# ORNL/MultiDistTorch

Measured on AMD Instinct MI355X. Metric: aggregate VAE samples/sec across K concurrent HPO trials, higher is better.
Workload: dtype bf16; 1 GPU; model=conv-VAE 28x28 (2 conv + 2 deconv, z=32), global_batch=128, per_trial_batch=128, image=28, parallelism=groups1x1, trials=1, backend=hip, graphs=True, timing_barrier=none, valid=True

## Files before the change

csrc/kernels/common.h:

```cpp
#pragma once
#include <hip/hip_runtime.h>
#include <stdint.h>

namespace mdt {

typedef float f32x4 __attribute__((ext_vector_type(4)));
typedef float f32x16 __attribute__((ext_vector_type(16)));

constexpr int kWave = 64;

__device__ __forceinline__ int lane_id() { return threadIdx.x & 63; }
__device__ __forceinline__ int wave_id() { return threadIdx.x >> 6; }

__device__ __forceinline__ f32x4 mfma16x16x4(float a, float b, f32x4 c) {
  return __builtin_amdgcn_mfma_f32_16x16x4f32(a, b, c, 0, 0, 0);
}

__device__ __forceinline__ f32x16 mfma32x32x2(float a, float b, f32x16 c) {
  return __builtin_amdgcn_mfma_f32_32x32x2f32(a, b, c, 0, 0, 0);
}

__device__ __forceinline__ float wave_sum(float v) {
#pragma unroll
  for (int o = 32; o > 0; o >>= 1) v += __shfl_xor(v, o, 64);
// ... 43 lines not shown
#pragma clang fp contract(off)
  return 1.f + lv - mu * mu - sd * sd;
}
__device__ __forceinline__ bool fb_clamped(float sum, float fb) { return fb > 0.f && -0.5f * sum < fb; }
__device__ __forceinline__ float fb_fwd(float sum, float fb) { return fb_clamped(sum, fb) ? -2.f * fb : sum; }
__device__ __forceinline__ float fb_bwd(float sum, float fb, float beta) { return fb_clamped(sum, fb) ? 0.f : beta; }

__device__ __forceinline__ float kl_dmu(float dz, float be, float mu) { return fmaf(be, mu, dz); }
__device__ __forceinline__ float kl_dlv(float dz, float ep, float sd, float be) {
  return fmaf(sd, 0.5f * dz * ep, 0.5f * be * fmaf(sd, sd, -1.f));
}
__device__ __forceinline__ float kl_dlv_sum(float dz, float ep, float sd, float be) {
  return fmaf(0.5f * be, fmaf(sd, sd, -1.f), 0.5f * dz * ep * sd);
}

__device__ __forceinline__ void st_wt8(void* p, unsigned long long v) {
  __hip_atomic_store(reinterpret_cast<unsigned long long*>(p), v, __ATOMIC_RELAXED, __HIP_MEMORY_SCOPE_AGENT);
}

__device__ __forceinline__ bool p2p_wait_abandoned(const int* status, const int* abort_flag, int lane) {
  int bad = 0;
  if (lane == 0) {
    bad = __hip_atomic_load(status, __ATOMIC_RELAXED, __HIP_MEMORY_SCOPE_SYSTEM) != 0;
    if (!bad && abort_flag) bad = __hip_atomic_load(abort_flag, __ATOMIC_RELAXED, __HIP_MEMORY_SCOPE_SYSTEM) != 0;
  }
  return __any(bad);
}

}
```

csrc/kernels/conv28_pair.h:

```cpp
#pragma once
#include <stddef.h>

#include "conv28_fused.h"

namespace mdt {
namespace f28 {

struct PairCtl {
  unsigned long long* xg;
  int* pairw;
  unsigned* err;
  int M;
  int pair;
  int delay_us;
  int acquire;
  AdamC* adamc;
};

constexpr int kX1 = 0, kX2 = 72, kX3 = kX2 + 800, kX4 = kX3 + 784, kX5 = kX4 + 1568, kX6 = kX5 + 32;
constexpr int kXW = kX6 + 800;
constexpr unsigned long long kSpinTicks = 25000000ull;

enum : int { kModeSolo = 0, kModeRole0 = 1, kModeRole1 = 2, kModeExit = 3 };

// ... 41 lines not shown
    if (!__any(pend != 0)) break;
    if ((spin & 15) == 15 && __builtin_amdgcn_s_memrealtime() - t0 > kSpinTicks) {
      if (pend) atomicOr(err, 1u);
      break;
    }
    __builtin_amdgcn_s_sleep(1);
  }
#pragma unroll
  for (int k = 0; k < N; ++k)
    if (gi[k] >= 0) {
      if (near && MDT_F28_NEAR_WG)
        __hip_atomic_store((g64*)(base + gi[k]), 0ull, __ATOMIC_RELAXED, __HIP_MEMORY_SCOPE_WORKGROUP);
      else
        __hip_atomic_store((g64*)(base + gi[k]), 0ull, __ATOMIC_RELAXED, __HIP_MEMORY_SCOPE_AGENT);
    }
}

using kseg = const __attribute__((address_space(4))) char;
__device__ __forceinline__ kseg* kargs() {
  kseg* k = (kseg*)__builtin_amdgcn_kernarg_segment_ptr();
  asm volatile("" : "+s"(k));
  return k;
}

template <class T>
__device__ __forceinline__ T kval(size_t off) {
  return *(const __attribute__((address_space(4))) T*)(kargs() + off);
}

template <class T>
__device__ __forceinline__ T* kptr(size_t off, size_t stride = 0, int n = 0) {
  const unsigned long long v = kval<unsigned long long>(off);
  auto* g = (__attribute__((address_space(1))) T*)(v ? v + stride * (unsigned long long)n : 0ull);
  return (T*)g;
}
#define F28_KP(T, member, stride) kptr<T>(offsetof(StepKargs, member), (stride), n)

__device__ __forceinline__ uint32_t fbits(float f) { return __builtin_bit_cast(uint32_t, f); }
__device__ __forceinline__ float bitsf(uint32_t u) { return __builtin_bit_cast(float, u); }
__device__ __forceinline__ uint32_t bf16bits(__bf16 h) { return (uint32_t)__builtin_bit_cast(uint16_t, h); }

template <class BFrag, class Pre, class Epi>
// ... 667 lines not shown
```

csrc/kernels/conv_bf16.hip:

```cpp
#include <stdlib.h>
#include "common.h"
#include "vae_mlp.h"
#include "adam_common.h"
#include "conv_igemm.h"
#include "conv_small.h"

namespace mdt {

__global__ void __launch_bounds__(256) reparam_k(const float* mulv, float* eps, __bf16* z16, float* z32, int B,
                                                 int Z, const TrainState* st, const HParams* hp, uint32_t stream,
                                                 float* kld_part) {
  __shared__ float scratch[16];
  const int e = blockIdx.x * blockDim.x + threadIdx.x;
  float kl = 0.f;
  if (e < B * Z) {
    const int i = e / Z, c = e - i * Z;
    const float mu = mulv[(size_t)i * 2 * Z + c], lv = mulv[(size_t)i * 2 * Z + Z + c];
    const long long stp = st->step - 1;
    const float fb = st->fb_t;
    const u32x4 bits = philox4x32_10(u32x4{(uint32_t)(i * Z + c), stream, (uint32_t)((unsigned long long)stp & 0xffffffffu),
                                           (uint32_t)((unsigned long long)stp >> 32)},
                                     hp->seed_lo, hp->seed_hi);
    const float ep = normal_from_bits(bits.x, bits.y);
    const float sd = expf(0.5f * lv);
// ... 196 lines not shown
int mdt_adam_cast(float* P, const float* G, float* Mo, float* Vo, void* w16, const void* segs, int nseg,
                  long long total, const void* st, const void* hp, int do_adam, hipStream_t s) {
  (void)segs;
  (void)nseg;
  if (total % 4 || ((uintptr_t)P | (uintptr_t)G | (uintptr_t)Mo | (uintptr_t)Vo) % 16 || (uintptr_t)w16 % 8) return 1;
  int blocks = cdivh(total / 4, 256);
  if (blocks > 1024) blocks = 1024;
  if (blocks < 1) blocks = 1;
  hipLaunchKernelGGL(adam_cast_k, dim3(blocks), dim3(256), 0, s, P, G, Mo, Vo, reinterpret_cast<__bf16*>(w16), total,
                     reinterpret_cast<const TrainState*>(st), reinterpret_cast<const HParams*>(hp), do_adam);
  return (int)hipGetLastError();
}

int mdt_grad_finalize(float* P, float* G, float* Mo, float* Vo, void* w16, const void* segs, const void* units,
                      int nunits, const void* st, const void* hp, int do_adam, const float* gX, const int* gidx,
                      float* xn, unsigned* xtag, int gB, hipStream_t s) {
  if (nunits <= 0) return 0;
  const FinalizeArgs fa{P, G, Mo, Vo, reinterpret_cast<__bf16*>(w16), reinterpret_cast<const GradSeg*>(segs),
                        reinterpret_cast<const GradUnit*>(units), reinterpret_cast<const TrainState*>(st),
                        reinterpret_cast<const HParams*>(hp), do_adam};
  const bool gather = xn && xtag && gX && gidx && gB > 0;
  const BatchGather bg{gX, gidx, reinterpret_cast<const TrainState*>(st), gather ? xn : nullptr, xtag, gB, nunits};
  const int grid = nunits + (gather ? gather_blocks(gB) : 0);
  static const bool fence = [] {
    const char* e = getenv("MDT_FIN_FENCE");
    return e && e[0] == '1';
  }();
  if (fence)
    hipLaunchKernelGGL(grad_finalize_k<true>, dim3(grid), dim3(kFinalizeThreads), 0, s, fa, bg);
  else
    hipLaunchKernelGGL(grad_finalize_k<false>, dim3(grid), dim3(kFinalizeThreads), 0, s, fa, bg);
  return (int)hipGetLastError();
}

int mdt_wtrans(const void* w16, void* w16t, const void* segs, const void* units, int nunits, hipStream_t s) {
// ... 29 lines not shown
```

csrc/kernels/conv_jobs.hip:

```cpp
#include <string.h>

#include <algorithm>

#include "conv_direct.h"
#include "conv_dwgrad.h"
#include "conv_igemm_dev.h"
#include "comm_jobs.h"
#include "conv_small.h"
#include "conv_thin.h"
#include "conv_thin_wg.h"

namespace mdt {
using namespace tiles;

struct JobPack {
  JobBlob j[3];
  int start1, start2;
};

template <class T>
__device__ __forceinline__ const T& job_args(const JobBlob& j) {
  return *reinterpret_cast<const T*>(j.args);
}

// ... 133 lines not shown
    case kJobWgradAdam:
      wgrad_body<__bf16, true, W0, true>(job_args<WgAdamArgs>(j).w, lds, lb, j.nblk, &job_args<WgAdamArgs>(j));
      break;
    case kJobWgradAdam + 1:
      wgrad_body<__bf16, true, W1, true>(job_args<WgAdamArgs>(j).w, lds, lb, j.nblk, &job_args<WgAdamArgs>(j));
      break;
    case kJobLossStep: JLossStep::run(j, lds, lb); break;
    case kJobLoss: JLoss::run(j, lds, lb); break;
    case kJobFinalize: JFinalize::run(j, lds, lb); break;
    case kJobComm: JComm::run(j, lds, lb); break;
    case kJobColsum: JColsum::run(j, lds, lb); break;
    default: break;
  }
}

__global__ void __launch_bounds__(256) jobs_multi_k(const JobPackN* __restrict__ p) {
  __shared__ __attribute__((aligned(16))) uint8_t lds[kMultiLds];
  const int b = blockIdx.x;
  int st[kMaxMultiJobs];
#pragma unroll
  for (int k = 0; k < kMaxMultiJobs; ++k) st[k] = p->start[k];
  const int n = p->n;
  int i = 0, s0 = st[0];
#pragma unroll
  for (int k = 1; k < kMaxMultiJobs; ++k)
    if (k < n && b >= st[k]) {
      i = k;
      s0 = st[k];
    }
  unsigned long long* stamps = p->stamps;
  unsigned long long t0 = 0;
  if (stamps) t0 = __builtin_amdgcn_s_memrealtime();
  run_multi_job(p->j[i], lds, b - s0);
  if (stamps) {
    __syncthreads();
    if (threadIdx.x == 0) {
      stamps[2 * b] = t0;
      stamps[2 * b + 1] = __builtin_amdgcn_s_memrealtime();
    }
  }
}

__host__ inline bool multi_kind_ok(int k) {
  if (k >= kJobWgrad && k <= kJobWgrad + 5) return true;
  if (k >= kJobWgradThin && k <= kJobWgradThin + 5) return true;
  if (k >= kJobWgradThin + 20 && k <= kJobWgradThin + 25) return true;
  if (k == kJobWgradAdam || k == kJobWgradAdam + 1) return true;
  return k == kJobLossStep || k == kJobLoss || k == kJobFinalize || k == kJobColsum || k == kJobComm;
}

template <class A, class B, class C>
__global__ void __launch_bounds__(256) jobs_k(JobPack p) {
  __shared__ __attribute__((aligned(1024))) uint8_t lds[cmax(cmax(A::LDS, B::LDS), cmax(C::LDS, 16))];
  const int b = blockIdx.x;
  if (b < p.start1) A::run(p.j[0], lds, b);
// ... 226 lines not shown
  return 0;
}

int mdt_job_loss(JobBlob* j, const float* bce_part, int nb, const float* kld_part, int nk, void* st, const void* hp,
                 int advance_cursor) {
  memset(j, 0, sizeof(*j));
  j->kind = (advance_cursor & 2) ? kJobLossStep : kJobLoss;
  advance_cursor &= 1;
  j->nblk = 1;
  put_args(j, LossArgs{bce_part, nb, kld_part, nk, reinterpret_cast<TrainState*>(st),
                       reinterpret_cast<const HParams*>(hp), advance_cursor});
  return 0;
}

int mdt_job_finalize(JobBlob* j, float* P, float* G, float* Mo, float* Vo, void* w16, const void* segs,
                     const void* units, int nunits, const void* st, const void* hp, int do_adam) {
  memset(j, 0, sizeof(*j));
  if (nunits <= 0) return 1;
  j->kind = kJobFinalize;
  j->nblk = nunits;
  put_args(j, FinalizeArgs{P, G, Mo, Vo, reinterpret_cast<__bf16*>(w16), reinterpret_cast<const GradSeg*>(segs),
                           reinterpret_cast<const GradUnit*>(units), reinterpret_cast<const TrainState*>(st),
                           reinterpret_cast<const HParams*>(hp), do_adam});
  return 0;
}

int mdt_job_comm(JobBlob* j, float* P, float* G, float* Mo, float* Vo, void* w16, const void* segs, const void* units,
                 int nunits, const void* st, const void* hp, int do_adam, const void* ctx, int mode) {
  memset(j, 0, sizeof(*j));
  if (nunits <= 0 || !ctx || mode < kCommPush || mode > kCommPushReduce) return 1;
  j->kind = kJobComm;
  j->nblk = nunits;
  CommJobArgs a{};
  a.fa = FinalizeArgs{P, G, Mo, Vo, reinterpret_cast<__bf16*>(w16), reinterpret_cast<const GradSeg*>(segs),
                      reinterpret_cast<const GradUnit*>(units), reinterpret_cast<const TrainState*>(st),
                      reinterpret_cast<const HParams*>(hp), do_adam};
  a.ctx = reinterpret_cast<const CommCtx*>(ctx);
  a.mode = mode;
  put_args(j, a);
  return 0;
}

int mdt_job_wtrans(JobBlob* j, const void* w16, void* w16t, const void* segs, const void* units, int nunits) {
  memset(j, 0, sizeof(*j));
  if (nunits <= 0) return 1;
  j->kind = kJobWtrans;
  j->nblk = nunits;
  put_args(j, WtransArgs{reinterpret_cast<const __bf16*>(w16), reinterpret_cast<__bf16*>(w16t),
                         reinterpret_cast<const GradSeg*>(segs), reinterpret_cast<const TrUnit*>(units)});
  return 0;
}
// ... 40 lines not shown
    p.start[i] = grid;
    grid += jobs[i].nblk;
  }
  p.start[n] = grid;
  p.n = n;
  memcpy(dst, &p, sizeof(p));
  return grid;
}

int mdt_launch_jobs_multi(const void* dev_pack, int grid, hipStream_t s) {
  if (!dev_pack || grid <= 0) return 2;
  hipLaunchKernelGGL(jobs_multi_k, dim3(grid), dim3(256), 0, s, reinterpret_cast<const JobPackN*>(dev_pack));
  return (int)hipGetLastError() ? -1 : 0;
}

int mdt_launch_job1(const JobBlob* j, hipStream_t s) {
  if (j->kind == kJobCombine) return launch_splitk_combine(*reinterpret_cast<const CombineArgs*>(j->args), j->nblk, s);
  return 1;
}

}
```

csrc/kernels/conv_small.h:

```cpp
#pragma once
#include "adam_common.h"
#include "common.h"
#include "conv_igemm.h"
#include "vae_mlp.h"

namespace mdt {

struct LossArgs {
  const float* bce_part;
  int nb;
  const float* kld_part;
  int nk;
  TrainState* st;
  const HParams* hp;
  int advance_cursor;
};

__device__ __forceinline__ void loss_finalize_body(const LossArgs& la, float* scratch) {
  float sb = 0.f, sk = 0.f;
  for (int i = threadIdx.x; i < la.nb; i += blockDim.x) sb += la.bce_part[i];
  for (int i = threadIdx.x; i < la.nk; i += blockDim.x) sk += la.kld_part[i];
  const float bce = block_sum(sb, scratch);
  __syncthreads();
  const float kld = block_sum(sk, scratch);
// ... 240 lines not shown
  a.dmulv[(size_t)i * 2 * a.Z + a.Z + c] = dl;
  if (a.dmulv16) {
    a.dmulv16[(size_t)i * 2 * a.Z + c] = (__bf16)dm;
    a.dmulv16[(size_t)i * 2 * a.Z + a.Z + c] = (__bf16)dl;
  }
}

struct FinalizeArgs {
  float *P, *G, *Mo, *Vo;
  __bf16* w16;
  const GradSeg* segs;
  const GradUnit* units;
  const TrainState* st;
  const HParams* hp;
  int do_adam;
};

constexpr int kFinalizeThreads = 256;

struct BatchGather {
  const float* X;
  const int* idx;
  const TrainState* st;
  float* xn;
  unsigned* xtag;
  int B, nunits;
};
__host__ __device__ constexpr int gather_blocks(int B) { return (B * 196 + kFinalizeThreads - 1) / kFinalizeThreads; }

__device__ __forceinline__ void batch_gather_body(const BatchGather& g, int b) {
// ... 86 lines not shown
    if (sg.slab) {
      g = slab_sum1(sg.slab + e0 + j, n, sg.nsplit);
      if (!a.do_adam) a.G[o + j] = g;
    } else {
      g = a.G[o + j];
    }
    if (a.do_adam) {
      float p = a.P[o + j], m = a.Mo[o + j], v = a.Vo[o + j];
      adam_update(p, m, v, g, c);
      a.P[o + j] = p; a.Mo[o + j] = m; a.Vo[o + j] = v;
      a.w16[o + j] = (__bf16)p;
    }
  }
}

__device__ __forceinline__ void grad_finalize_body(const FinalizeArgs& a, float* red, AdamC* cs, int bid) {
  AdamC c{};
  if (a.do_adam) c = adam_consts_block(a.st, a.hp, cs);
  const GradUnit u = a.units[bid];
  const GradSeg sg = a.segs[u.seg];
  if (u.count > kFinalizeThreads) {
    grad_finalize_vec4(a, c, u, sg);
    return;
  }
  const int t = threadIdx.x, cnt = u.count, rp = kFinalizeThreads / cnt;
  const int col = t % cnt, rl = t / cnt;
  float part = 0.f;
  if (sg.slab && rl < rp) part = slab_partial(sg.slab + u.start + col, sg.numel, sg.nsplit, rl, rp);
  red[t] = part;
  __syncthreads();
  if (rl == 0) {
    const long long o = sg.off + u.start + col;
    float g;
    if (sg.slab) {
      g = 0.f;
// ... 71 lines not shown
```

csrc/runtime/conv_ops.cpp:

```cpp
#include <torch/extension.h>
#include <c10/hip/HIPStream.h>
#include <ATen/hip/impl/HIPGuardImplMasqueradingAsCUDA.h>

#include <cmath>
#include <cstring>
#include <tuple>
#include <vector>

#include "../kernels/vae_mlp.h"

#include "../kernels/conv_igemm.h"

extern "C" {
int mdt_igemm_plan(int mode, mdt::ConvDesc d, int allow_split, int* info, int fwd);
void mdt_dconv_stamps(unsigned long long* p);
int mdt_wgrad_plan(mdt::ConvDesc d, int* info);
int mdt_igemm(int mode, const void* A, int a_is_f32, const void* B16, mdt::ConvDesc d, const float* bias, int relu,
              void* y16, float* y32, const void* omask, float* colsum, float* ws, int skip_combine, hipStream_t s,
              const mdt::APro* pro, int fwd);
int mdt_wgrad(const void* G16, const void* X, int x_is_f32, mdt::ConvDesc d, float* out, hipStream_t s);
int mdt_colsum(const void* G16, int M, int N, int rows_per, float* slab, hipStream_t s);
int mdt_gather_rows(const float* X, const int* idx, const void* st, int B, int M, int P, float* xb, hipStream_t s);
int mdt_reparam(const float* mulv, float* eps, void* z16, float* z32, int B, int Z, const void* st, const void* hp,
                unsigned stream, float* kld_part, hipStream_t s);
int mdt_reparam_bwd(const float* dz, const float* mulv, const float* eps, float* dmulv, void* dmulv16, int B, int Z,
                    const float* klw, const float* fbw, hipStream_t s);
int mdt_bce_logits(const float* logits, const float* X, const int* rows, int B, int P, void* dlog16, float* recon,
                   float* part, float* gpart, hipStream_t s);
int mdt_conv_loss_finalize(const float* bce_part, int nb, const float* kld_part, int nk, void* st, const void* hp,
                           int advance_cursor, hipStream_t s);
int mdt_step_begin(void* st, const void* hp, hipStream_t s);
int mdt_adam_cast(float* P, const float* G, float* Mo, float* Vo, void* w16, const void* segs, int nseg,
                  long long total, const void* st, const void* hp, int do_adam, hipStream_t s);
int mdt_grad_finalize(float* P, float* G, float* Mo, float* Vo, void* w16, const void* segs, const void* units,
                      int nunits, const void* st, const void* hp, int do_adam, const float* gX, const int* gidx,
                      float* xn, unsigned* xtag, int gB, hipStream_t s);
int mdt_wtrans(const void* w16, void* w16t, const void* segs, const void* units, int nunits, hipStream_t s);
int mdt_thin_conv(const void* X, int x_is_f32, const float* Wf, mdt::ConvDesc d, const float* bias, int relu, void* y16,
                  const void* omask, float* colsum, const int* idx, void* st, const void* hp, int B, float* xb,
                  hipStream_t s);
int mdt_thin_blocks(int tconv, mdt::ConvDesc d);
int mdt_thin_tconv(const void* G16, const float* Wf, mdt::ConvDesc d, const float* bias, float* y32, const float* X,
                   void* dlog16, float* recon, float* part, float* gpart, hipStream_t s);
int mdt_job_igemm(mdt::JobBlob* g, mdt::JobBlob* c, int mode, const void* A, int a_is_f32, const void* B16,
                  mdt::ConvDesc d, const float* bias, int relu, void* y16, float* y32, const void* omask,
                  float* colsum, float* ws, int skip_combine);
int mdt_job_finalize(mdt::JobBlob* j, float* P, float* G, float* Mo, float* Vo, void* w16, const void* segs,
                     const void* units, int nunits, const void* st, const void* hp, int do_adam);
int mdt_job_wtrans(mdt::JobBlob* j, const void* w16, void* w16t, const void* segs, const void* units, int nunits);
int mdt_job_comm(mdt::JobBlob* j, float* P, float* G, float* Mo, float* Vo, void* w16, const void* segs,
                 const void* units, int nunits, const void* st, const void* hp, int do_adam, const void* ctx, int mode);
int mdt_combine_reparam(const float* slab, int ks, const float* bias, float* mulv, float* eps, void* z16, float* z32,
                        int B, int Z, const void* st, const void* hp, unsigned stream, float* kld_part, hipStream_t s);
int mdt_combine_reparam_blocks(int ks, int B, int Z);
int mdt_combine_reparam_bwd(const float* slab, int ks, const float* mulv, const float* eps, float* dmulv,
                            void* dmulv16, float* dz, int B, int Z, const float* klw, const float* fbw,
                            hipStream_t s);
int mdt_job_wgrad(mdt::JobBlob* j, const void* G16, const void* X, int x_is_f32, mdt::ConvDesc d, float* out);
int mdt_job_wgrad_adam(mdt::JobBlob* j, const void* G16, const void* X, int x_is_f32, mdt::ConvDesc d, float* P,
                       float* Mo, float* Vo, void* w16, const float* adamc);
int mdt_job_thin_conv(mdt::JobBlob* j, const void* X, int x_is_f32, const float* Wf, mdt::ConvDesc d,
                      const float* bias, int relu, void* y16, const void* omask, float* colsum, const int* idx,
                      void* st, const void* hp, int B, float* xb);
int mdt_job_colsum(mdt::JobBlob* j, const void* G16, int M, int N, int rows_per, float* slab);
int mdt_job_loss(mdt::JobBlob* j, const float* bce_part, int nb, const float* kld_part, int nk, void* st,
                 const void* hp, int advance_cursor);
int mdt_launch_jobs(const mdt::JobBlob* jobs, int n, hipStream_t s);
int mdt_jobs_multi_bytes();
int mdt_pack_jobs_multi(const mdt::JobBlob* jobs, int n, void* dst);
int mdt_pack_jobs_multi_stamps(void* img, void* stamps);
int mdt_launch_jobs_multi(const void* dev_pack, int grid, hipStream_t s);
int mdt_f28_forward(const long long* p, int B, int M, unsigned stream, int train, hipStream_t s);
int mdt_f28_forward_pair(const long long* p, const long long* pp, int B, int M, unsigned stream, hipStream_t s);
int mdt_f28_backward(const long long* p, int M, const void* st, hipStream_t s);
int mdt_f28_step(const long long* pf, const long long* pb, const long long* pp, int B, int M, unsigned stream,
                 int pair, int delay_us, float* adamc, hipStream_t s);
int mdt_f28_pair_words();
int mdt_launch_job1(const mdt::JobBlob* j, hipStream_t s);
}

namespace mdt {

struct Job {
  JobBlob main{}, post{};
  int kind() const { return main.kind; }
  bool has_post() const { return post.kind != 0; }
// ... 373 lines not shown
    TORCH_CHECK(j != nullptr && !j->has_post(), "pack_jobs_multi: null job or job with a follow-up pass");
    TORCH_CHECK(j->main.kind > 0, "pack_jobs_multi: job has no fused form (kind 0)");
    v.push_back(j->main);
  }
  auto img = torch::zeros({(int64_t)mdt_jobs_multi_bytes()}, torch::kUInt8);
  const int grid = mdt_pack_jobs_multi(v.data(), (int)v.size(), img.data_ptr());
  TORCH_CHECK(grid > 0, "pack_jobs_multi: unsupported job kind or bad job (", grid, ")");
  if (stamps.has_value() && stamps->defined()) {
    TORCH_CHECK(stamps->is_cuda() && stamps->scalar_type() == torch::kInt64 && stamps->numel() >= 2 * grid,
                "pack_jobs_multi: stamps must be an int64 CUDA tensor of >= 2 * grid elements");
    mdt_pack_jobs_multi_stamps(img.data_ptr(), stamps->data_ptr());
  }
  return {img, (int64_t)grid};
}

void launch_jobs_multi(const at::Tensor& dev_pack, int64_t grid) {
  TORCH_CHECK(dev_pack.is_cuda() && dev_pack.scalar_type() == torch::kUInt8 &&
                  dev_pack.numel() >= mdt_jobs_multi_bytes(), "launch_jobs_multi: device job table");
  const int r = mdt_launch_jobs_multi(dev_pack.data_ptr(), (int)grid, cur());
  TORCH_CHECK(r == 0, "mdt: launch_jobs_multi failed (", r, ")");
}

namespace {
struct Slot {
  const char* name;
  char dtype;
  int64_t per_m;
  bool fixed;
  bool optional;
};

std::vector<long long> f28_ptrs(const std::vector<c10::optional<at::Tensor>>& t, const std::vector<Slot>& slots,
                                int64_t M, int dev) {
  TORCH_CHECK(t.size() <= slots.size(), "f28: expected ", slots.size(), " tensors, got ", t.size());
// ... 173 lines not shown
  check_buf(P, torch::kFloat32, total, P, "adam_cast", "P");
  check_buf(G, torch::kFloat32, total, P, "adam_cast", "G");
  check_buf(M, torch::kFloat32, total, P, "adam_cast", "m");
  check_buf(V, torch::kFloat32, total, P, "adam_cast", "v");
  check_buf(w16, torch::kBFloat16, total, P, "adam_cast", "w16");
  check_blob(state, sizeof(TrainState), P, "adam_cast", "state");
  check_blob(hparams, sizeof(HParams), P, "adam_cast", "hparams");
  rc(mdt_adam_cast(P.data_ptr<float>(), G.data_ptr<float>(), M.data_ptr<float>(), V.data_ptr<float>(),
                   w16.data_ptr(), segs.data_ptr(), (int)nseg, P.numel(), state.data_ptr(), hparams.data_ptr(),
                   do_adam ? 1 : 0, cur()),
     "adam_cast");
}

void grad_finalize(at::Tensor P, at::Tensor G, at::Tensor M, at::Tensor V, at::Tensor w16, const at::Tensor& segs,
                   const at::Tensor& units, int64_t nunits, const at::Tensor& state, const at::Tensor& hparams,
                   bool do_adam, Job* job, const std::vector<at::Tensor>& gather, int64_t gather_B) {
  TORCH_CHECK(units.numel() >= nunits * (int64_t)sizeof(GradUnit), "grad_finalize: unit table too small");
  if (job) {
    TORCH_CHECK(gather.empty(), "grad_finalize: a finalize job takes no gather");
    rc(mdt_job_finalize(&job->main, P.data_ptr<float>(), G.data_ptr<float>(), M.data_ptr<float>(),
                        V.data_ptr<float>(), w16.data_ptr(), segs.data_ptr(), units.data_ptr(), (int)nunits,
                        state.data_ptr(), hparams.data_ptr(), do_adam ? 1 : 0),
       "job_finalize");
    return;
  }
  const float* gX = nullptr;
  const int* gidx = nullptr;
  float* xn = nullptr;
  unsigned* xtag = nullptr;
  if (!gather.empty()) {
    TORCH_CHECK(gather.size() == 4 && gather_B > 0, "grad_finalize: gather = [X, idx, xn, xtag] with gather_B > 0");
    const int dev = P.get_device();
    const char* nm[4] = {"X", "idx", "xn", "xtag"};
    for (int i = 0; i < 4; ++i)
      TORCH_CHECK(gather[i].is_cuda() && gather[i].get_device() == dev && gather[i].is_contiguous(),
                  "grad_finalize: gather ", nm[i], " must be a contiguous tensor on the arena's device");
    TORCH_CHECK(gather[0].scalar_type() == torch::kFloat32 && gather[0].numel() % 784 == 0, "grad_finalize: X [rows][784] f32");
    TORCH_CHECK(gather[1].scalar_type() == torch::kInt32 && gather[1].numel() % gather_B == 0,
                "grad_finalize: idx int32 in whole batches");
    TORCH_CHECK(gather[2].scalar_type() == torch::kFloat32 && gather[2].numel() >= gather_B * 784, "grad_finalize: xn");
    TORCH_CHECK(gather[3].scalar_type() == torch::kInt32 && gather[3].numel() >= gather_B, "grad_finalize: xtag");
    gX = gather[0].data_ptr<float>();
    gidx = gather[1].data_ptr<int>();
    xn = gather[2].data_ptr<float>();
    xtag = reinterpret_cast<unsigned*>(gather[3].data_ptr<int>());
  }
  rc(mdt_grad_finalize(P.data_ptr<float>(), G.data_ptr<float>(), M.data_ptr<float>(), V.data_ptr<float>(),
                       w16.data_ptr(), segs.data_ptr(), units.data_ptr(), (int)nunits, state.data_ptr(),
                       hparams.data_ptr(), do_adam ? 1 : 0, gX, gidx, xn, xtag, (int)gather_B, cur()),
     "grad_finalize");
}

void comm_job(at::Tensor P, at::Tensor G, at::Tensor M, at::Tensor V, at::Tensor w16, const at::Tensor& segs,
              const at::Tensor& units, int64_t nunits, const at::Tensor& state, const at::Tensor& hparams,
              bool do_adam, int64_t ctx, int64_t mode, Job* job) {
  TORCH_CHECK(job != nullptr, "comm_job: records into a Job (no stand-alone launch)");
  TORCH_CHECK(units.numel() >= nunits * (int64_t)sizeof(GradUnit), "comm_job: unit table too small");
  TORCH_CHECK(P.numel() == G.numel() && M.numel() == G.numel() && V.numel() == G.numel() && w16.numel() == G.numel(),
              "comm_job: arenas differ in size");
  rc(mdt_job_comm(&job->main, P.data_ptr<float>(), G.data_ptr<float>(), M.data_ptr<float>(), V.data_ptr<float>(),
                  w16.data_ptr(), segs.data_ptr(), units.data_ptr(), (int)nunits, state.data_ptr(),
                  hparams.data_ptr(), do_adam ? 1 : 0, reinterpret_cast<const void*>((intptr_t)ctx), (int)mode),
     "job_comm");
}
// ... 62 lines not shown
      TORCH_CHECK(t->is_cuda() && t->scalar_type() == torch::kInt64, "dconv_stamps: int64 CUDA tensor");
      mdt_dconv_stamps(reinterpret_cast<unsigned long long*>(t->data_ptr()));
    } else {
      mdt_dconv_stamps(nullptr);
    }
  });
  m.def("wgrad_plan", &wgrad_plan);
  py::class_<Job>(m, "Job")
      .def(py::init<>())
      .def_property_readonly("kind", &Job::kind)
      .def_property_readonly("nblk", [](const Job& j) { return j.main.nblk; })
      .def_property_readonly("has_post", &Job::has_post);
  m.def("launch_jobs", &launch_jobs);
  m.def("pack_jobs_multi", &pack_jobs_multi, py::arg("jobs"), py::arg("stamps") = py::none());
  m.def("launch_jobs_multi", &launch_jobs_multi, py::arg("dev_pack"), py::arg("grid"));
  m.def("f28_forward", &f28_forward, py::arg("tensors"), py::arg("B"), py::arg("M"), py::arg("stream"),
        py::arg("train"), py::arg("pair") = std::vector<c10::optional<at::Tensor>>{});
  m.def("f28_backward", &f28_backward, py::arg("tensors"), py::arg("M"), py::arg("state") = py::none());
  m.def("f28_pair_words", &mdt_f28_pair_words);
  m.def("f28_step", &f28_step, py::arg("fwd_tensors"), py::arg("bwd_tensors"), py::arg("B"), py::arg("M"),
        py::arg("stream"), py::arg("pair") = std::vector<c10::optional<at::Tensor>>{},
        py::arg("pair_delay_us") = 0, py::arg("adamc") = py::none());
  m.def("igemm", &igemm, py::arg("mode"), py::arg("A"), py::arg("B16"), py::arg("desc"), py::arg("bias"),
        py::arg("relu"), py::arg("y16"), py::arg("y32"), py::arg("omask") = py::none(),
        py::arg("colsum") = py::none(), py::arg("ws") = py::none(), py::arg("job") = py::none(),
        py::arg("combine") = true, py::arg("a_slab") = py::none(), py::arg("a_ks") = 0,
        py::arg("a_bias") = py::none(), py::arg("a_relu") = false, py::arg("a_out16") = py::none(),
        py::arg("fwd") = false);
  m.def("wgrad", &wgrad, py::arg("G16"), py::arg("X"), py::arg("desc"), py::arg("out"), py::arg("job") = py::none(),
        py::arg("adam") = std::vector<at::Tensor>{}, py::arg("adam_off") = 0, py::arg("adamc") = py::none());
// ... 16 lines not shown
  m.def("loss_finalize2", &loss_finalize2, py::arg("bce_part"), py::arg("nb"), py::arg("kld_part"), py::arg("nk"),
        py::arg("state"), py::arg("hparams"), py::arg("advance_cursor"), py::arg("job") = py::none(),
        py::arg("advance_step") = false);
  m.def("step_begin", &step_begin);
  m.def("make_grad_segs", &make_grad_segs);
  m.def("make_grad_units", &make_grad_units);
  m.def("make_tr_units", &make_tr_units);
  m.def("adam_cast", &adam_cast);
  m.def("graph_upload", [](int64_t exec) {
    TORCH_CHECK(exec != 0, "graph_upload: null graph exec");
    rc((int)hipGraphUpload(reinterpret_cast<hipGraphExec_t>((intptr_t)exec), cur()), "hipGraphUpload");
  });
  m.def("grad_finalize", &grad_finalize, py::arg("P"), py::arg("G"), py::arg("M"), py::arg("V"), py::arg("w16"),
        py::arg("segs"), py::arg("units"), py::arg("nunits"), py::arg("state"), py::arg("hparams"),
        py::arg("do_adam"), py::arg("job") = py::none(), py::arg("gather") = std::vector<at::Tensor>{},
        py::arg("gather_B") = 0);
  m.def("comm_job", &comm_job, py::arg("P"), py::arg("G"), py::arg("M"), py::arg("V"), py::arg("w16"),
        py::arg("segs"), py::arg("units"), py::arg("nunits"), py::arg("state"), py::arg("hparams"),
        py::arg("do_adam"), py::arg("ctx"), py::arg("mode"), py::arg("job"));
  m.def("wtrans", &wtrans, py::arg("w16"), py::arg("w16t"), py::arg("segs"), py::arg("units"), py::arg("nunits"),
        py::arg("job") = py::none());
  m.def("combine_reparam", &combine_reparam);
  m.def("combine_reparam_bwd", &combine_reparam_bwd, py::arg("ws"), py::arg("ks"), py::arg("mulv"), py::arg("eps"),
        py::arg("dmulv"), py::arg("dmulv16"), py::arg("dz"), py::arg("B"), py::arg("Z"), py::arg("hparams"),
        py::arg("state") = py::none());
  m.def("combine_reparam_blocks", &mdt_combine_reparam_blocks);
}

}
```

multidisttorch_amd/models/conv28.py:

```python

import math
import os

import torch

from ..ops.conv_plans import wgrad_plan
from .conv_spec import _w_shape
from .trainer_base import EVAL_STREAM


class Fused28Step:
    def _init28(self):
        self.f28 = (self.backend == "hip" and self.image == 28 and self.channels == 1 and self.Z == 32
                    and os.getenv("MDT_CONV_F28", "1") != "0" and not self.tc_on)
        self._plans28 = {}
        self.f28_skip_adam = False
        self.f28_merge = os.getenv("MDT_F28_MERGE", "1") != "0"
        self.f28_pair = os.getenv("MDT_F28_PAIR", "1") != "0"
        self._eval_pair = os.getenv("MDT_F28_EVAL_PAIR", "1") != "0"
        self.f28_pair_delay_us = -int(os.getenv("MDT_F28_TEST_STALL_US", "0"))
        self.f28_stamps = (None, None)

    def _alloc28(self):
        B, dev = self.B, self.device
        f32 = dict(dtype=torch.float32, device=dev)
        self.dlog32 = torch.zeros(B * self.D, **f32)
        self.f28_part = torch.zeros(3 * B, **f32)
        self.f28_bias = torch.zeros(B * (3136 + 32 + 128 + 32), **f32)
        self.f28_xg = torch.zeros(B * 2 * self.C.f28_pair_words(), dtype=torch.int64, device=dev)
        self.f28_pairw = torch.zeros(B, dtype=torch.int32, device=dev)
        self.f28_err = torch.zeros(1, dtype=torch.int32, device=dev)
        self.f28_xn = torch.zeros(B * self.D, **f32)
        self.f28_xtag = torch.full((B,), -1, dtype=torch.int32, device=dev)
        self.f28_prefetch = os.getenv("MDT_F28_PREFETCH", "1") != "0"
        self.f28_epi_adam = os.getenv("MDT_F28_EPI_ADAM", "1") != "0"
        self.f28_adamc = torch.zeros(16, **f32)

    def _invalidate_prefetch(self):
        xt = getattr(self, "f28_xtag", None)
        if xt is not None:
            xt.fill_(-1)

    def _health28(self):
        msgs = []
        err = int(self.f28_err.item())
        if err:
            msgs.append(f"fused 28x28 step: a paired-workgroup exchange timed out (f28_err={err}); "
                        f"the trial trained on incomplete partial sums")
        return msgs

    def _plan28(self, M):
# ... 22 lines not shown
        slabs, jobs = {}, []
        for name, (G, Xw) in srcs.items():
            l = self.by_name[name]
            d = self._desc(l, M)
            ns = wgrad_plan(d).nsplit
            t = torch.empty(ns * math.prod(_w_shape(l)), **f32)
            slabs[name + ".weight"] = (t, ns)
            jobs.append(self._job(lambda j: C.wgrad(G, Xw, d, t, job=j)))
        jobs.append(self._job(lambda j: C.loss_finalize2(bce, M, kld, M, st.train_state, st.hparams, True, job=j,
                                                         advance_step=True)))
        for name, t, rows in (("enc1", db1, M), ("enc2", db2, 2 * M), ("enc_head", self.dmulv, M),
                              ("dec_fc", dbd, M), ("dec1", db3, M), ("dec2", db4, M)):
            slabs[name + ".bias"] = (t, rows)
        segs = self._seg_rows(slabs)
        units, layer_units = self._finalize_units(segs)
        pack, grid = C.pack_jobs_multi(jobs)
        names = list(srcs)
        dec_jobs = [jobs[i] for i, n in enumerate(names) if n.startswith("dec")] + [jobs[len(names)]]
        enc_jobs = [jobs[i] for i, n in enumerate(names) if not n.startswith("dec")]
        dec_pack, dec_grid = C.pack_jobs_multi(dec_jobs)
        enc_pack, enc_grid = C.pack_jobs_multi(enc_jobs)
        first_dec = self.spec.index(self.dec[0])
        p = dict(fwd=fwd, bwd=bwd, jobs=jobs, jobs_pack=pack.to(dev), jobs_grid=grid, slabs=slabs,
                 segs=C.make_grad_segs(segs, dev.index or 0), units=C.make_grad_units(units, dev.index or 0),
                 nunits=len(units), layer_units=layer_units, first_dec=first_dec,
                 dec_pack=dec_pack.to(dev), dec_grid=dec_grid, enc_pack=enc_pack.to(dev), enc_grid=enc_grid,
                 dec_jobs=dec_jobs, enc_jobs=enc_jobs, names=names)
        p["epi_src"] = (M, srcs, segs, units)
        self._plans28[M] = p
        return p

    _EPI_ADAM28 = ("enc_head", "dec_fc")

    def _epi_plan28(self, p):
        if "epi" not in p:
            p["epi"] = self._build_epi_plan28(p, *p["epi_src"])
        return p["epi"]

    def _build_epi_plan28(self, p, M, srcs, segs, units):
        C, dev = self.C, self.device
        seg_of = {l.name: 2 * i for i, l in enumerate(self.spec)}
        for n in self._EPI_ADAM28:
            if p["slabs"][n + ".weight"][1] != 1 or segs[seg_of[n]][0] % 4 or segs[seg_of[n]][1] % 4:
                return None
        jobs = list(p["jobs"])
        for n in self._EPI_ADAM28:
            G, Xw = srcs[n]
            jobs[p["names"].index(n)] = self._job(lambda j: C.wgrad(
                G, Xw, self._desc(self.by_name[n], M), p["slabs"][n + ".weight"][0], job=j,
                adam=[self.params, self.exp_avg, self.exp_avg_sq, self.w16], adam_off=segs[seg_of[n]][0],
                adamc=self.f28_adamc))
        skip = {seg_of[n] for n in self._EPI_ADAM28}
        eunits = [u for u in units if u[0] not in skip]
        pack, grid = C.pack_jobs_multi(jobs)
        return dict(jobs=jobs, jobs_pack=pack.to(dev), jobs_grid=grid,
                    units=C.make_grad_units(eunits, dev.index or 0), nunits=len(eunits))

    def _step28(self, M):
        C, p, st = self.C, self._plan28(M), self.state
        red = self.reducer
        epi = (self._epi_plan28(p) if self.f28_epi_adam and red is None and self.f28_merge
               and not self.f28_skip_adam else None)
        if self.f28_merge:
            C.f28_step(p["fwd"], p["bwd"], self.B, M, self.rng_stream,
                       pair=[self.f28_xg, self.f28_pairw, self.f28_err] if self.f28_pair else [],
                       pair_delay_us=self.f28_pair_delay_us, **({"adamc": self.f28_adamc} if epi else {}))
        else:
            C.f28_forward(p["fwd"], self.B, M, self.rng_stream, True)
            C.f28_backward(p["bwd"], M, state=st.train_state)
        if red is None:
            q = epi or p
            C.launch_jobs_multi(q["jobs_pack"], q["jobs_grid"])
            self._grad_finalize(p["segs"], q["units"], 0, q["nunits"], not self.f28_skip_adam,
                                gather=([self._data[0], self._data[1], self.f28_xn, self.f28_xtag]
                                        if self.f28_prefetch else []), gather_B=self.B)
            return
        if self._comm_ctx():
            packs = self._comm_packs28(M, p)
            for i, (pack, grid) in enumerate(packs):
                C.launch_jobs_multi(pack, grid)
                if self.comm_phase_hook is not None and i == len(packs) - 2:
                    self.comm_phase_hook()
            return
        lu, fd, L = p["layer_units"], p["first_dec"], len(self.spec)
        dec0 = self.layer_ranges()[fd][1]
        bounds = list(red.bounds())
        nbk = len(bounds) - 1
        early = self._overlap28(fused=False)
        if hasattr(red, "set_inline"):
            red.set_inline(not early)
        if not early:
            C.launch_jobs_multi(p["jobs_pack"], p["jobs_grid"])
            self._finalize_unit_range(p, lu[0], lu[L])
            for k in reversed(range(nbk)):
                red.launch(k)
        else:
            C.launch_jobs_multi(p["dec_pack"], p["dec_grid"])
            self._finalize_unit_range(p, lu[fd], lu[L])
            for k in reversed(range(nbk)):
                if bounds[k] >= dec0:
                    red.launch(k)
            C.launch_jobs_multi(p["enc_pack"], p["enc_grid"])
            self._finalize_unit_range(p, lu[0], lu[fd])
            for k in reversed(range(nbk)):
                if bounds[k] < dec0:
                    red.launch(k)
        red.wait_all()
        if not self.f28_skip_adam:
            self._adam_cast(True)

    def _comm_packs28(self, M, p):
        adam = not self.f28_skip_adam
        overlap = self._overlap28(fused=True) and not self.comm_split_tail
        key = (M, adam, overlap, self.comm_split_tail)
        packs = self._comm_packs.get(key)
        if packs is not None:
            return packs
        C, dev = self.C, self.device
        lu, fd, L = p["layer_units"], p["first_dec"], len(self.spec)
        segs, units = p["segs"], p["units"]
        jobs = p["jobs"]
        enc, dec = p["enc_jobs"], p["dec_jobs"]
        if self.comm_split_tail:
            tables = [jobs, [self._comm_job(segs, units, lu[0], lu[L], 1, adam)],
                      [self._comm_job(segs, units, lu[0], lu[L], 2, adam)]]
        elif overlap:
            tables = [dec,
                      enc + [self._comm_job(segs, units, lu[fd], lu[L], 1, adam)],
                      [self._comm_job(segs, units, lu[0], lu[fd], 3, adam),
                       self._comm_job(segs, units, lu[fd], lu[L], 2, adam)]]
        else:
            tables = [jobs, [self._comm_job(segs, units, lu[0], lu[L], 3, adam)]]
        self._comm_tables[key] = tables
        packs = []
        for i, t in enumerate(tables):
            st = self.comm_stamps[i] if self.comm_stamps is not None and i < len(self.comm_stamps) else None
            pack, grid = C.pack_jobs_multi(t, stamps=st)
            packs.append((pack.to(dev), grid))
        self._comm_packs[key] = packs
        return packs

    def _overlap28(self, fused: bool) -> bool:
        if self.ddp_overlap is not None:
            return bool(self.ddp_overlap)
        from ..parallel.ddp import overlap_pays

        return overlap_pays(4 * (self.numel - self.split), 6.0 if fused else 31.0)

    def _finalize_unit_range(self, p, u0, u1):
        if u1 > u0:
            self._grad_finalize(p["segs"], p["units"], u0, u1, False)

    def _f28_weights(self):
# ... 21 lines not shown
```

Before: 2.298 million samples/s.

## Pass multi-job table by value in kernargs, reuse Adam constants, lane-cache grad segments

Adds a jobs_multi_kv kernel that receives the whole job pack by value in the kernel-argument segment, so blocks read job descriptors from kernarg memory instead of a device buffer. By default it launches from a host copy of the pack. The grad-finalize kernel can now take precomputed Adam constants instead of recomputing them per block, and it loads the segment table across wave lanes and picks entries with readlane rather than doing a dependent global load. The aim is to cut global-memory latency on small, latency-bound kernels. The cost is a larger kernarg payload per launch, which graph capture must snapshot.

```diff
diff --git a/csrc/kernels/common.h b/csrc/kernels/common.h
--- a/csrc/kernels/common.h
+++ b/csrc/kernels/common.h
@@ -81,6 +81,18 @@
   return fmaf(0.5f * be, fmaf(sd, sd, -1.f), 0.5f * dz * ep * sd);
 }
 
+using kseg = const __attribute__((address_space(4))) char;
+__device__ __forceinline__ kseg* kargs() {
+  kseg* k = (kseg*)__builtin_amdgcn_kernarg_segment_ptr();
+  asm volatile("" : "+s"(k));
+  return k;
+}
+
+template <class T>
+__device__ __forceinline__ T kval(size_t off) {
+  return *(const __attribute__((address_space(4))) T*)(kargs() + off);
+}
+
 __device__ __forceinline__ void st_wt8(void* p, unsigned long long v) {
   __hip_atomic_store(reinterpret_cast<unsigned long long*>(p), v, __ATOMIC_RELAXED, __HIP_MEMORY_SCOPE_AGENT);
 }
diff --git a/csrc/kernels/conv28_pair.h b/csrc/kernels/conv28_pair.h
--- a/csrc/kernels/conv28_pair.h
+++ b/csrc/kernels/conv28_pair.h
@@ -79,18 +79,6 @@
       else
         __hip_atomic_store((g64*)(base + gi[k]), 0ull, __ATOMIC_RELAXED, __HIP_MEMORY_SCOPE_AGENT);
     }
-}
-
-using kseg = const __attribute__((address_space(4))) char;
-__device__ __forceinline__ kseg* kargs() {
-  kseg* k = (kseg*)__builtin_amdgcn_kernarg_segment_ptr();
-  asm volatile("" : "+s"(k));
-  return k;
-}
-
-template <class T>
-__device__ __forceinline__ T kval(size_t off) {
-  return *(const __attribute__((address_space(4))) T*)(kargs() + off);
 }
 
 template <class T>
diff --git a/csrc/kernels/conv_bf16.hip b/csrc/kernels/conv_bf16.hip
--- a/csrc/kernels/conv_bf16.hip
+++ b/csrc/kernels/conv_bf16.hip
@@ -234,11 +234,11 @@
 
 int mdt_grad_finalize(float* P, float* G, float* Mo, float* Vo, void* w16, const void* segs, const void* units,
                       int nunits, const void* st, const void* hp, int do_adam, const float* gX, const int* gidx,
-                      float* xn, unsigned* xtag, int gB, hipStream_t s) {
+                      float* xn, unsigned* xtag, int gB, int nsegs, const float* adamc, hipStream_t s) {
   if (nunits <= 0) return 0;
   const FinalizeArgs fa{P, G, Mo, Vo, reinterpret_cast<__bf16*>(w16), reinterpret_cast<const GradSeg*>(segs),
                         reinterpret_cast<const GradUnit*>(units), reinterpret_cast<const TrainState*>(st),
-                        reinterpret_cast<const HParams*>(hp), do_adam};
+                        reinterpret_cast<const HParams*>(hp), do_adam, nsegs, reinterpret_cast<const AdamC*>(adamc)};
   const bool gather = xn && xtag && gX && gidx && gB > 0;
   const BatchGather bg{gX, gidx, reinterpret_cast<const TrainState*>(st), gather ? xn : nullptr, xtag, gB, nunits};
   const int grid = nunits + (gather ? gather_blocks(gB) : 0);
diff --git a/csrc/kernels/conv_jobs.hip b/csrc/kernels/conv_jobs.hip
--- a/csrc/kernels/conv_jobs.hip
+++ b/csrc/kernels/conv_jobs.hip
@@ -171,7 +171,10 @@
   }
 }
 
-__global__ void __launch_bounds__(256) jobs_multi_k(const JobPackN* __restrict__ p) {
+static_assert(sizeof(JobPackN) <= 4096, "jobs_multi_kv passes the pack by value: the kernel-argument segment limit");
+
+template <bool KV, class P>
+__device__ __forceinline__ void jobs_multi_body(P p) {
   __shared__ __attribute__((aligned(16))) uint8_t lds[kMultiLds];
   const int b = blockIdx.x;
   int st[kMaxMultiJobs];
@@ -185,17 +188,36 @@
       i = k;
       s0 = st[k];
     }
-  unsigned long long* stamps = p->stamps;
-  unsigned long long t0 = 0;
-  if (stamps) t0 = __builtin_amdgcn_s_memrealtime();
-  run_multi_job(p->j[i], lds, b - s0);
-  if (stamps) {
-    __syncthreads();
-    if (threadIdx.x == 0) {
-      stamps[2 * b] = t0;
-      stamps[2 * b + 1] = __builtin_amdgcn_s_memrealtime();
+  if constexpr (KV) {
+    if (unsigned long long* stamps = p->stamps) {
+      if (threadIdx.x == 0) stamps[2 * b] = __builtin_amdgcn_s_memrealtime();
     }
-  }
+    run_multi_job(*(const JobBlob*)(const void*)&p->j[i], lds, b - s0);
+    P q = p;
+    asm volatile("" : "+s"(q));
+    if (unsigned long long* stamps = q->stamps) {
+      __syncthreads();
+      if (threadIdx.x == 0) stamps[2 * blockIdx.x + 1] = __builtin_amdgcn_s_memrealtime();
+    }
+  } else {
+    unsigned long long* stamps = p->stamps;
+    unsigned long long t0 = 0;
+    if (stamps) t0 = __builtin_amdgcn_s_memrealtime();
+    run_multi_job(*(const JobBlob*)(const void*)&p->j[i], lds, b - s0);
+    if (stamps) {
+      __syncthreads();
+      if (threadIdx.x == 0) {
+        stamps[2 * b] = t0;
+        stamps[2 * b + 1] = __builtin_amdgcn_s_memrealtime();
+      }
+    }
+  }
+}
+
+__global__ void __launch_bounds__(256) jobs_multi_k(const JobPackN* __restrict__ p) { jobs_multi_body<false>(p); }
+
+__global__ void __launch_bounds__(256) jobs_multi_kv(JobPackN) {
+  jobs_multi_body<true>((const __attribute__((address_space(4))) JobPackN*)kargs());
 }
 
 __host__ inline bool multi_kind_ok(int k) {
@@ -452,14 +474,16 @@
 }
 
 int mdt_job_finalize(JobBlob* j, float* P, float* G, float* Mo, float* Vo, void* w16, const void* segs,
-                     const void* units, int nunits, const void* st, const void* hp, int do_adam) {
+                     const void* units, int nunits, const void* st, const void* hp, int do_adam, int nsegs,
+                     const float* adamc) {
   memset(j, 0, sizeof(*j));
   if (nunits <= 0) return 1;
   j->kind = kJobFinalize;
   j->nblk = nunits;
   put_args(j, FinalizeArgs{P, G, Mo, Vo, reinterpret_cast<__bf16*>(w16), reinterpret_cast<const GradSeg*>(segs),
                            reinterpret_cast<const GradUnit*>(units), reinterpret_cast<const TrainState*>(st),
-                           reinterpret_cast<const HParams*>(hp), do_adam});
+                           reinterpret_cast<const HParams*>(hp), do_adam, nsegs,
+                           reinterpret_cast<const AdamC*>(adamc)});
   return 0;
 }
 
@@ -472,7 +496,7 @@
   CommJobArgs a{};
   a.fa = FinalizeArgs{P, G, Mo, Vo, reinterpret_cast<__bf16*>(w16), reinterpret_cast<const GradSeg*>(segs),
                       reinterpret_cast<const GradUnit*>(units), reinterpret_cast<const TrainState*>(st),
-                      reinterpret_cast<const HParams*>(hp), do_adam};
+                      reinterpret_cast<const HParams*>(hp), do_adam, 0, nullptr};
   a.ctx = reinterpret_cast<const CommCtx*>(ctx);
   a.mode = mode;
   put_args(j, a);
@@ -543,6 +567,15 @@
   return (int)hipGetLastError() ? -1 : 0;
 }
 
+int mdt_launch_jobs_multi_host(const void* host_pack, int grid, hipStream_t s) {
+  if (!host_pack || grid <= 0) return 2;
+  JobPackN p;
+  memcpy(&p, host_pack, sizeof(p));
+  if (p.n < 1 || p.n > kMaxMultiJobs || p.start[p.n] != grid) return 2;
+  hipLaunchKernelGGL(jobs_multi_kv, dim3(grid), dim3(256), 0, s, p);
+  return (int)hipGetLastError() ? -1 : 0;
+}
+
 int mdt_launch_job1(const JobBlob* j, hipStream_t s) {
   if (j->kind == kJobCombine) return launch_splitk_combine(*reinterpret_cast<const CombineArgs*>(j->args), j->nblk, s);
   return 1;
diff --git a/csrc/kernels/conv_small.h b/csrc/kernels/conv_small.h
--- a/csrc/kernels/conv_small.h
+++ b/csrc/kernels/conv_small.h
@@ -278,6 +278,8 @@
   const TrainState* st;
   const HParams* hp;
   int do_adam;
+  int nsegs;
+  const AdamC* adamc;
 };
 
 constexpr int kFinalizeThreads = 256;
@@ -394,11 +396,49 @@
   }
 }
 
+struct SegLanes {
+  static constexpr int NW = sizeof(GradSeg) / 4;
+  static_assert(sizeof(GradSeg) % 8 == 0 && alignof(GradSeg) == 8, "a GradSeg moves as 8-B words");
+  uint32_t w[NW];
+};
+
+__device__ __forceinline__ SegLanes finalize_seg_load(const GradSeg* segs, int nsegs, int l) {
+  typedef uint32_t u32x2 __attribute__((ext_vector_type(2)));
+  SegLanes r;
+#pragma unroll
+  for (int k = 0; k < SegLanes::NW; ++k) r.w[k] = 0u;
+  if (l < nsegs) {
+    const u32x2* s = reinterpret_cast<const u32x2*>(segs + l);
+#pragma unroll
+    for (int k = 0; k < SegLanes::NW / 2; ++k) {
+      const u32x2 v = s[k];
+      r.w[2 * k] = v[0];
+      r.w[2 * k + 1] = v[1];
+    }
+  }
+  return r;
+}
+
+__device__ __forceinline__ GradSeg finalize_seg_pick(const SegLanes& v, int seg) {
+  const int sl = __builtin_amdgcn_readfirstlane(seg);
+  uint32_t r[SegLanes::NW];
+#pragma unroll
+  for (int k = 0; k < SegLanes::NW; ++k) r[k] = (uint32_t)__builtin_amdgcn_readlane((int)v.w[k], sl);
+  GradSeg sg;
+  __builtin_memcpy(&sg, r, sizeof(sg));
+  return sg;
+}
+
 __device__ __forceinline__ void grad_finalize_body(const FinalizeArgs& a, float* red, AdamC* cs, int bid) {
   AdamC c{};
-  if (a.do_adam) c = adam_consts_block(a.st, a.hp, cs);
+  const bool lanes = a.nsegs > 0 && a.nsegs <= kWave;
+  SegLanes sv{};
+  if (lanes) sv = finalize_seg_load(a.segs, a.nsegs, lane_id());
+  const bool handed = a.do_adam && a.adamc != nullptr;
+  if (a.do_adam && !handed) c = adam_consts_block(a.st, a.hp, cs);
   const GradUnit u = a.units[bid];
-  const GradSeg sg = a.segs[u.seg];
+  if (handed) c = *a.adamc;
+  const GradSeg sg = lanes ? finalize_seg_pick(sv, u.seg) : a.segs[u.seg];
   if (u.count > kFinalizeThreads) {
     grad_finalize_vec4(a, c, u, sg);
     return;
diff --git a/csrc/runtime/conv_ops.cpp b/csrc/runtime/conv_ops.cpp
--- a/csrc/runtime/conv_ops.cpp
+++ b/csrc/runtime/conv_ops.cpp
@@ -34,7 +34,7 @@
                   long long total, const void* st, const void* hp, int do_adam, hipStream_t s);
 int mdt_grad_finalize(float* P, float* G, float* Mo, float* Vo, void* w16, const void* segs, const void* units,
                       int nunits, const void* st, const void* hp, int do_adam, const float* gX, const int* gidx,
-                      float* xn, unsigned* xtag, int gB, hipStream_t s);
+                      float* xn, unsigned* xtag, int gB, int nsegs, const float* adamc, hipStream_t s);
 int mdt_wtrans(const void* w16, void* w16t, const void* segs, const void* units, int nunits, hipStream_t s);
 int mdt_thin_conv(const void* X, int x_is_f32, const float* Wf, mdt::ConvDesc d, const float* bias, int relu, void* y16,
                   const void* omask, float* colsum, const int* idx, void* st, const void* hp, int B, float* xb,
@@ -46,7 +46,8 @@
                   mdt::ConvDesc d, const float* bias, int relu, void* y16, float* y32, const void* omask,
                   float* colsum, float* ws, int skip_combine);
 int mdt_job_finalize(mdt::JobBlob* j, float* P, float* G, float* Mo, float* Vo, void* w16, const void* segs,
-                     const void* units, int nunits, const void* st, const void* hp, int do_adam);
+                     const void* units, int nunits, const void* st, const void* hp, int do_adam, int nsegs,
+                     const float* adamc);
 int mdt_job_wtrans(mdt::JobBlob* j, const void* w16, void* w16t, const void* segs, const void* units, int nunits);
 int mdt_job_comm(mdt::JobBlob* j, float* P, float* G, float* Mo, float* Vo, void* w16, const void* segs,
                  const void* units, int nunits, const void* st, const void* hp, int do_adam, const void* ctx, int mode);
@@ -70,6 +71,7 @@
 int mdt_pack_jobs_multi(const mdt::JobBlob* jobs, int n, void* dst);
 int mdt_pack_jobs_multi_stamps(void* img, void* stamps);
 int mdt_launch_jobs_multi(const void* dev_pack, int grid, hipStream_t s);
+int mdt_launch_jobs_multi_host(const void* host_pack, int grid, hipStream_t s);
 int mdt_f28_forward(const long long* p, int B, int M, unsigned stream, int train, hipStream_t s);
 int mdt_f28_forward_pair(const long long* p, const long long* pp, int B, int M, unsigned stream, hipStream_t s);
 int mdt_f28_backward(const long long* p, int M, const void* st, hipStream_t s);
@@ -473,10 +475,11 @@
   return {img, (int64_t)grid};
 }
 
-void launch_jobs_multi(const at::Tensor& dev_pack, int64_t grid) {
-  TORCH_CHECK(dev_pack.is_cuda() && dev_pack.scalar_type() == torch::kUInt8 &&
-                  dev_pack.numel() >= mdt_jobs_multi_bytes(), "launch_jobs_multi: device job table");
-  const int r = mdt_launch_jobs_multi(dev_pack.data_ptr(), (int)grid, cur());
+void launch_jobs_multi(const at::Tensor& pack, int64_t grid) {
+  TORCH_CHECK(pack.scalar_type() == torch::kUInt8 && pack.is_contiguous() && pack.numel() >= mdt_jobs_multi_bytes(),
+              "launch_jobs_multi: job table (pack_jobs_multi's image, or a device copy of it)");
+  const int r = pack.is_cuda() ? mdt_launch_jobs_multi(pack.data_ptr(), (int)grid, cur())
+                               : mdt_launch_jobs_multi_host(pack.data_ptr(), (int)grid, cur());
   TORCH_CHECK(r == 0, "mdt: launch_jobs_multi failed (", r, ")");
 }
 
@@ -680,13 +683,18 @@
 
 void grad_finalize(at::Tensor P, at::Tensor G, at::Tensor M, at::Tensor V, at::Tensor w16, const at::Tensor& segs,
                    const at::Tensor& units, int64_t nunits, const at::Tensor& state, const at::Tensor& hparams,
-                   bool do_adam, Job* job, const std::vector<at::Tensor>& gather, int64_t gather_B) {
+                   bool do_adam, Job* job, const std::vector<at::Tensor>& gather, int64_t gather_B,
+                   const c10::optional<at::Tensor>& adamc) {
   TORCH_CHECK(units.numel() >= nunits * (int64_t)sizeof(GradUnit), "grad_finalize: unit table too small");
+  const int64_t nsegs64 = segs.numel() / (int64_t)sizeof(GradSeg);
+  const int nsegs = nsegs64 <= 64 ? (int)nsegs64 : 0;
+  const float* ac = nullptr;
+  if (adamc.has_value() && adamc->defined()) ac = adamc_ptr(*adamc, P.get_device(), "grad_finalize");
   if (job) {
     TORCH_CHECK(gather.empty(), "grad_finalize: a finalize job takes no gather");
     rc(mdt_job_finalize(&job->main, P.data_ptr<float>(), G.data_ptr<float>(), M.data_ptr<float>(),
                         V.data_ptr<float>(), w16.data_ptr(), segs.data_ptr(), units.data_ptr(), (int)nunits,
-                        state.data_ptr(), hparams.data_ptr(), do_adam ? 1 : 0),
+                        state.data_ptr(), hparams.data_ptr(), do_adam ? 1 : 0, nsegs, ac),
        "job_finalize");
     return;
   }
@@ -713,7 +721,7 @@
   }
   rc(mdt_grad_finalize(P.data_ptr<float>(), G.data_ptr<float>(), M.data_ptr<float>(), V.data_ptr<float>(),
                        w16.data_ptr(), segs.data_ptr(), units.data_ptr(), (int)nunits, state.data_ptr(),
-                       hparams.data_ptr(), do_adam ? 1 : 0, gX, gidx, xn, xtag, (int)gather_B, cur()),
+                       hparams.data_ptr(), do_adam ? 1 : 0, gX, gidx, xn, xtag, (int)gather_B, nsegs, ac, cur()),
      "grad_finalize");
 }
 
@@ -806,6 +814,7 @@
   m.def("launch_jobs", &launch_jobs);
   m.def("pack_jobs_multi", &pack_jobs_multi, py::arg("jobs"), py::arg("stamps") = py::none());
   m.def("launch_jobs_multi", &launch_jobs_multi, py::arg("dev_pack"), py::arg("grid"));
+  m.def("jobs_multi_bytes", [] { return (int64_t)mdt_jobs_multi_bytes(); });
   m.def("f28_forward", &f28_forward, py::arg("tensors"), py::arg("B"), py::arg("M"), py::arg("stream"),
         py::arg("train"), py::arg("pair") = std::vector<c10::optional<at::Tensor>>{});
   m.def("f28_backward", &f28_backward, py::arg("tensors"), py::arg("M"), py::arg("state") = py::none());
@@ -852,7 +861,7 @@
   m.def("grad_finalize", &grad_finalize, py::arg("P"), py::arg("G"), py::arg("M"), py::arg("V"), py::arg("w16"),
         py::arg("segs"), py::arg("units"), py::arg("nunits"), py::arg("state"), py::arg("hparams"),
         py::arg("do_adam"), py::arg("job") = py::none(), py::arg("gather") = std::vector<at::Tensor>{},
-        py::arg("gather_B") = 0);
+        py::arg("gather_B") = 0, py::arg("adamc") = py::none());
   m.def("comm_job", &comm_job, py::arg("P"), py::arg("G"), py::arg("M"), py::arg("V"), py::arg("w16"),
         py::arg("segs"), py::arg("units"), py::arg("nunits"), py::arg("state"), py::arg("hparams"),
         py::arg("do_adam"), py::arg("ctx"), py::arg("mode"), py::arg("job"));
diff --git a/multidisttorch_amd/models/conv28.py b/multidisttorch_amd/models/conv28.py
--- a/multidisttorch_amd/models/conv28.py
+++ b/multidisttorch_amd/models/conv28.py
@@ -35,6 +35,7 @@
         self.f28_prefetch = os.getenv("MDT_F28_PREFETCH", "1") != "0"
         self.f28_epi_adam = os.getenv("MDT_F28_EPI_ADAM", "1") != "0"
         self.f28_adamc = torch.zeros(16, **f32)
+        self.f28_host_pack = self.f28_fin_adamc = hasattr(self.C, "jobs_multi_bytes")
 
     def _invalidate_prefetch(self):
         xt = getattr(self, "f28_xtag", None)
@@ -87,21 +88,29 @@
             slabs[name + ".bias"] = (t, rows)
         segs = self._seg_rows(slabs)
         units, layer_units = self._finalize_units(segs)
-        pack, grid = C.pack_jobs_multi(jobs)
+        host, pack, grid = self._pack28(jobs)
         names = list(srcs)
         dec_jobs = [jobs[i] for i, n in enumerate(names) if n.startswith("dec")] + [jobs[len(names)]]
         enc_jobs = [jobs[i] for i, n in enumerate(names) if not n.startswith("dec")]
-        dec_pack, dec_grid = C.pack_jobs_multi(dec_jobs)
-        enc_pack, enc_grid = C.pack_jobs_multi(enc_jobs)
+        dec_host, dec_pack, dec_grid = self._pack28(dec_jobs)
+        enc_host, enc_pack, enc_grid = self._pack28(enc_jobs)
         first_dec = self.spec.index(self.dec[0])
-        p = dict(fwd=fwd, bwd=bwd, jobs=jobs, jobs_pack=pack.to(dev), jobs_grid=grid, slabs=slabs,
+        p = dict(fwd=fwd, bwd=bwd, jobs=jobs, jobs_host=host, jobs_pack=pack, jobs_grid=grid, slabs=slabs,
                  segs=C.make_grad_segs(segs, dev.index or 0), units=C.make_grad_units(units, dev.index or 0),
                  nunits=len(units), layer_units=layer_units, first_dec=first_dec,
-                 dec_pack=dec_pack.to(dev), dec_grid=dec_grid, enc_pack=enc_pack.to(dev), enc_grid=enc_grid,
+                 dec_host=dec_host, dec_pack=dec_pack, dec_grid=dec_grid,
+                 enc_host=enc_host, enc_pack=enc_pack, enc_grid=enc_grid,
                  dec_jobs=dec_jobs, enc_jobs=enc_jobs, names=names)
         p["epi_src"] = (M, srcs, segs, units)
         self._plans28[M] = p
         return p
+
+    def _pack28(self, jobs, stamps=None):
+        pack, grid = self.C.pack_jobs_multi(jobs, stamps=stamps)
+        return pack, pack.to(self.device), grid
+
+    def _launch28(self, d, name="jobs"):
+        self.C.launch_jobs_multi(d[name + ("_host" if self.f28_host_pack else "_pack")], d[name + "_grid"])
 
     _EPI_ADAM28 = ("enc_head", "dec_fc")
 
@@ -125,8 +134,8 @@
                 adamc=self.f28_adamc))
         skip = {seg_of[n] for n in self._EPI_ADAM28}
         eunits = [u for u in units if u[0] not in skip]
-        pack, grid = C.pack_jobs_multi(jobs)
-        return dict(jobs=jobs, jobs_pack=pack.to(dev), jobs_grid=grid,
+        host, pack, grid = self._pack28(jobs)
+        return dict(jobs=jobs, jobs_host=host, jobs_pack=pack, jobs_grid=grid,
                     units=C.make_grad_units(eunits, dev.index or 0), nunits=len(eunits))
 
     def _step28(self, M):
@@ -143,10 +152,11 @@
             C.f28_backward(p["bwd"], M, state=st.train_state)
         if red is None:
             q = epi or p
-            C.launch_jobs_multi(q["jobs_pack"], q["jobs_grid"])
+            self._launch28(q)
             self._grad_finalize(p["segs"], q["units"], 0, q["nunits"], not self.f28_skip_adam,
                                 gather=([self._data[0], self._data[1], self.f28_xn, self.f28_xtag]
-                                        if self.f28_prefetch else []), gather_B=self.B)
+                                        if self.f28_prefetch else []), gather_B=self.B,
+                                **({"adamc": self.f28_adamc} if epi and self.f28_fin_adamc else {}))
             return
         if self._comm_ctx():
             packs = self._comm_packs28(M, p)
@@ -163,17 +173,17 @@
         if hasattr(red, "set_inline"):
             red.set_inline(not early)
         if not early:
-            C.launch_jobs_multi(p["jobs_pack"], p["jobs_grid"])
+            self._launch28(p)
             self._finalize_unit_range(p, lu[0], lu[L])
             for k in reversed(range(nbk)):
                 red.launch(k)
         else:
-            C.launch_jobs_multi(p["dec_pack"], p["dec_grid"])
+            self._launch28(p, "dec")
             self._finalize_unit_range(p, lu[fd], lu[L])
             for k in reversed(range(nbk)):
                 if bounds[k] >= dec0:
                     red.launch(k)
-            C.launch_jobs_multi(p["enc_pack"], p["enc_grid"])
+            self._launch28(p, "enc")
             self._finalize_unit_range(p, lu[0], lu[fd])
             for k in reversed(range(nbk)):
                 if bounds[k] < dec0:
@@ -185,11 +195,10 @@
     def _comm_packs28(self, M, p):
         adam = not self.f28_skip_adam
         overlap = self._overlap28(fused=True) and not self.comm_split_tail
-        key = (M, adam, overlap, self.comm_split_tail)
+        key = (M, adam, overlap, self.comm_split_tail, self.f28_host_pack)
         packs = self._comm_packs.get(key)
         if packs is not None:
             return packs
-        C, dev = self.C, self.device
         lu, fd, L = p["layer_units"], p["first_dec"], len(self.spec)
         segs, units = p["segs"], p["units"]
         jobs = p["jobs"]
@@ -204,12 +213,12 @@
                        self._comm_job(segs, units, lu[fd], lu[L], 2, adam)]]
         else:
             tables = [jobs, [self._comm_job(segs, units, lu[0], lu[L], 3, adam)]]
-        self._comm_tables[key] = tables
+        self._comm_tables[key[:4]] = tables
         packs = []
         for i, t in enumerate(tables):
             st = self.comm_stamps[i] if self.comm_stamps is not None and i < len(self.comm_stamps) else None
-            pack, grid = C.pack_jobs_multi(t, stamps=st)
-            packs.append((pack.to(dev), grid))
+            host, pack, grid = self._pack28(t, stamps=st)
+            packs.append((host if self.f28_host_pack else pack, grid))
         self._comm_packs[key] = packs
         return packs
 
```

After: 2.316 million samples/s (median of 6 runs). About the same (+0.8%).
